# UCSD-Comp-Imaging/Nerf-Simple

Hardware: NVIDIA B200
Metric: rays/sec (64 samples/ray) render (higher is better)
Workload: dtype bf16

## Files before the change

nerf_simple_b200/csrc/mlp_chain.cuh:

```cuda
constexpr uint32_t kC_A = 0, kC_E = 2 * kABytes, kC_W = kC_E + 2 * kEBytes;
constexpr int kCStages = 4;
constexpr uint32_t kCStageBytes = 16384;
constexpr uint32_t kC_Bar = kC_W + kCStages * kCStageBytes;
constexpr uint32_t kC_Bias = kC_Bar + 256;
constexpr uint32_t kCSmemLaunch = kC_Bias + 2 * 1024;
constexpr int kCThreads = 640;
constexpr int kCProducerWarp = 16, kCMmaWarp = 17, kCStoreWarp0 = 18;
constexpr uint32_t kB_WFull = 0, kB_WPeer = 32, kB_WEmpty = 64, kB_Act = 96, kB_Acc = 112, kB_Tmem = 128, kB_Written = 136,
                   kB_StoreFree = 152;

struct TileCtx {
  int64_t tile;
  int slot;
  int half;
  int part;
  uint32_t r;
  uint32_t rowoff;
  uint32_t r7s;
  uint32_t a_img, e_img, t_lane;
  uint32_t b_img;
  const float* gf;
};
__device__ __forceinline__ uint32_t sw_off(const TileCtx& c, uint32_t kb, uint32_t j) {
  return kb * 16384u + c.rowoff + ((j << 4) ^ c.r7s);
// ... 137 lines not shown

  const int64_t PT = (p.num_tiles + 1) / 2;
  const int64_t C = num_clusters_x(), cid = cluster_id_x();
  const int64_t my_pt = (cid < PT) ? (PT - cid + C - 1) / C : 0;
  const SlabDesc* slabs = Epi::slabs();

  if (warp < 16) {
    const int slot = Epi::kSlots == 2 ? warp >> 3 : 0;
    TileCtx c;
    c.slot = slot;
    c.half = (warp >> 2) & 1;
    c.part = warp >> 2;
    c.r = (uint32_t)(warp & 3) * 32u + (uint32_t)lane;
    c.rowoff = c.r * 128u;
    c.r7s = (c.r & 7u) << 4;
    c.a_img = smem_base + kC_A + slot * kABytes;
    c.e_img = smem_base + kC_E + slot * kEBytes;
    c.t_lane = tmem_base + (((uint32_t)(warp & 3) * 32u) << 16) + (uint32_t)slot * 256u;
    c.b_img = smem_base + kC_Bias + (uint32_t)slot * 1024u;
    c.gf = reinterpret_cast<const float*>(p.packed + (Epi::kSched == kSchedFwd3 ? c_layout.f32_off3 : c_layout.f32_off));
    const uint32_t act_remote = mapa_shared(bar + kB_Act + 8 * slot, 0);
    uint32_t acc_parity = 0, free_parity = 0;
    typename Epi::State st;
    bool first_step = true;
    long long t_epi = 0, t_accw = 0, t_pro = 0, t_reclaim = 0, t_after = 0, t_stage = 0;
    auto publish = [&](bool to_mma) {
      fence_proxy_async_smem();
      tc_fence_before();
      __syncwarp();
      if (lane == 0) {
        if (Epi::kBulkStore) mbar_arrive(bar + kB_Written + 8 * slot);
        if (to_mma) mbar_arrive_cluster(act_remote);
      }
    };
    const uint32_t bias_t = threadIdx.x & 255u;
    auto fetch_bias = [&](int l) -> float { return Epi::kStageBias ? __ldg(c.gf + kF32Bias + Epi::bias_row(l) * 256 + (int)bias_t) : 0.f; };
    auto stage_bias = [&](float v) {
      if (!Epi::kStageBias) return;
      if (Epi::kSlots == 2) slot_barrier(slot); else asm volatile("bar.sync 1, 512;" ::: "memory");
      if (Epi::kSlots == 2 || threadIdx.x < 256u) asm volatile("st.shared.f32 [%0], %1;" ::"r"(c.b_img + bias_t * 4u), "f"(v) : "memory");
      if (Epi::kSlots == 2) slot_barrier(slot); else asm volatile("bar.sync 1, 512;" ::: "memory");
    };
    auto reclaim = [&]() {
      if (Epi::kBulkStore && !first_step) {
        mbar_wait(bar + kB_StoreFree + 8 * slot, free_parity, 500);
        free_parity ^= 1;
      }
      first_step = false;
    };
    Epi::init_slot(c);
    for (int64_t k = slot; k < my_pt; k += Epi::kSlots) {
      c.tile = 2 * (cid + k * C) + rank;
      if (Epi::kReverseTiles) c.tile = 2 * (PT - 1 - (cid + k * C)) + rank;
      reclaim();
      long long tq0 = 0;
      if constexpr (Epi::kHasDbg && kDevBuild) tq0 = clock64();
      const float bias0 = fetch_bias(0);
      Epi::begin_tile(p, st, c);
      publish(true);
      stage_bias(bias0);
      if constexpr (Epi::kHasDbg && kDevBuild) t_pro += clock64() - tq0;
      for (int l = 0; l < Epi::kNumLayers; ++l) {
        Epi::prefetch(p, st, c, l);
        if constexpr (Epi::kHasDbg && kDevBuild) tq0 = clock64();
        mbar_wait(bar + kB_Acc + 8 * slot, acc_parity, 100 + l);
        acc_parity ^= 1;
        tc_fence_after();
        long long tq1 = 0;
        if constexpr (Epi::kHasDbg && kDevBuild) { tq1 = clock64(); t_accw += tq1 - tq0; }
        reclaim();
        if constexpr (Epi::kHasDbg && kDevBuild) t_reclaim += clock64() - tq1;
        const float bias_next = fetch_bias(l + 1 < Epi::kNumLayers ? l + 1 : l);
        Epi::layer(p, st, c, l);
        if (Epi::kBulkStore || l + 1 < Epi::kNumLayers) publish(l + 1 < Epi::kNumLayers);
        if constexpr (Epi::kHasDbg && kDevBuild) {
          const long long tq2 = clock64();
          t_epi += tq2 - tq1;
          if ((p.dbg & 8) && threadIdx.x == 0 && rank == 0 && p.dbg_counters) {
            atomicAdd(p.dbg_counters + 16 + l, (unsigned long long)(tq2 - tq1));
            atomicAdd(p.dbg_counters + 32 + l, (unsigned long long)(tq1 - tq0));
          }
        }
        long long tq3 = 0;
        if constexpr (Epi::kHasDbg && kDevBuild) tq3 = clock64();
        if (l + 1 < Epi::kNumLayers) stage_bias(bias_next);
        long long tq4 = 0;
        if constexpr (Epi::kHasDbg && kDevBuild) { tq4 = clock64(); t_stage += tq4 - tq3; }
        Epi::after_publish(p, st, c, l);
        if constexpr (Epi::kHasDbg && kDevBuild) t_after += clock64() - tq4;
      }
    }
    if constexpr (Epi::kHasDbg && kDevBuild) {
      if ((p.dbg & 8) && threadIdx.x == 0 && rank == 0 && p.dbg_counters) {
        atomicAdd(p.dbg_counters + 4, (unsigned long long)t_epi);
        atomicAdd(p.dbg_counters + 5, (unsigned long long)t_accw);
        atomicAdd(p.dbg_counters + 6, (unsigned long long)t_pro);
        atomicAdd(p.dbg_counters + 12, (unsigned long long)t_reclaim);
        atomicAdd(p.dbg_counters + 13, (unsigned long long)t_stage);
        atomicAdd(p.dbg_counters + 14, (unsigned long long)t_after);
      }
    }
    if (Epi::kBulkStore && !first_step) mbar_wait(bar + kB_StoreFree + 8 * slot, free_parity, 501);
  } else if (warp == kCProducerWarp) {
    if (lane == 0) {
      uint32_t stage = 0, phase = 0;
      long long t_pempty = 0;
      for (int64_t pr = 0; pr * Epi::kSlots < my_pt; ++pr) {
        const int nslots = (Epi::kSlots == 2 && my_pt - 2 * pr >= 2) ? 2 : 1;
        int s0 = 0;
        for (int l = 0; l < Epi::kNumLayers; ++l) {
          int s1 = s0;
          while (!slabs[s1].last) ++s1;
          const int reps = (nslots == 2 && s1 - s0 + 1 <= kCStages) ? 1 : nslots;
          for (int rep = 0; rep < reps; ++rep) {
            for (int s = s0; s <= s1; ++s) {
              const uint32_t half = slabs[s].bytes >> 1;
              if constexpr (Epi::kHasDbg && kDevBuild) {
                const long long tp0 = clock64();
                mbar_wait(bar + kB_WEmpty + 8 * stage, phase ^ 1, 200);
                const long long tp1 = clock64();
                t_pempty += tp1 - tp0;
              } else
              mbar_wait(bar + kB_WEmpty + 8 * stage, phase ^ 1, 200);
              if (rank == 0) mbar_arrive_expect_tx(bar + kB_WFull + 8 * stage, slabs[s].bytes);
              const int32_t row0 = (int32_t)(slabs[s].off >> 7) + (int32_t)(rank * (half >> 7));
              tma_tensor2d_g2s_2cta(smem_base + kC_W + stage * kCStageBytes, half == 16384u ? &p.tmap128 : &p.tmap64, 0, row0,
// ... 83 lines not shown
  int64_t num_tiles;
  float* rgb;
  float* disp;
  float* acc;
  int64_t B;
  int sampler;
  uint64_t seed, offset;
  float tn, tf;
  const float* poses;
  int H, W;
  float f;
  int64_t ray_begin;
};
constexpr int kInCamera = 2;

__device__ __forceinline__ void load_ray_chain(const FwdEpiParams& p, int64_t ray, float (&o)[6]) {
  if (p.in_mode == kInCamera) {
    camera_ray(p.poses, p.H, p.W, p.f, p.ray_begin + ray, o);
  } else {
    const float2* q = reinterpret_cast<const float2*>(p.in0 + ray * 6);
    const float2 a = __ldg(q), b = __ldg(q + 1), c = __ldg(q + 2);
    o[0] = a.x; o[1] = a.y; o[2] = b.x; o[3] = b.y; o[4] = c.x; o[5] = c.y;
  }
}

template <bool kRender>
__device__ __forceinline__ void load_query_chain(const FwdEpiParams& p, int64_t m, float v[6], float& t) {
  if (!kRender && p.in_mode == NB200_IN_POINTS) {
    const float2* q = reinterpret_cast<const float2*>(p.in0 + m * 6);
    const float2 a = __ldg(q), b = __ldg(q + 1), c = __ldg(q + 2);
    v[0] = a.x; v[1] = a.y; v[2] = b.x; v[3] = b.y; v[4] = c.x; v[5] = c.y;
    t = 0.f;
  } else {
    const int64_t ray = p.nshift >= 0 ? (m >> p.nshift) : m / p.N;
    float o[6];
    if (kRender) {
      load_ray_chain(p, ray, o);
      t = p.sampler ? philox_sample_depth(m, (int)(m - ray * p.N), p.N, p.tn, p.tf, p.seed, p.offset) : __ldg(p.in1 + m);
    } else {
      const float2* q = reinterpret_cast<const float2*>(p.in0 + ray * 6);
      const float2 a = __ldg(q), b = __ldg(q + 1), c = __ldg(q + 2);
      o[0] = a.x; o[1] = a.y; o[2] = b.x; o[3] = b.y; o[4] = c.x; o[5] = c.y;
      t = __ldg(p.in1 + m);
    }
    const float dx = o[3], dy = o[4], dz = o[5];
    v[0] = __fadd_rn(o[0], __fmul_rn(dx, t));
    v[1] = __fadd_rn(o[1], __fmul_rn(dy, t));
    v[2] = __fadd_rn(o[2], __fmul_rn(dz, t));
    const float inv = 1.0f / sqrtf(fmaf(dz, dz, fmaf(dy, dy, dx * dx)));
    v[3] = dx * inv; v[4] = dy * inv; v[5] = dz * inv;
  }
}

template <int S>
__device__ __forceinline__ void composite_staged_ray(const FwdEpiParams& p, uint32_t stage_o, uint32_t stage_t, int ray_local,
                                                     int64_t ray, int lane) {
  constexpr int N = 32 * S;
  float4 o[S];
  float t[S];
  const uint32_t row0 = (uint32_t)(ray_local * N + lane * S);
#pragma unroll
  for (int j = 0; j < S; ++j) {
    asm volatile("ld.shared.v4.f32 {%0,%1,%2,%3}, [%4];" : "=f"(o[j].x), "=f"(o[j].y), "=f"(o[j].z), "=f"(o[j].w) : "r"(stage_o + (row0 + j) * 16u));
    asm volatile("ld.shared.f32 %0, [%1];" : "=f"(t[j]) : "r"(stage_t + (row0 + j) * 4u));
  }
  float rd[6];
  load_ray_chain(p, ray, rd);
  const float norm = unit_dir_norm(rd[3], rd[4], rd[5]);
  const float t_next_lane = __shfl_down_sync(0xffffffffu, t[0], 1);
  float a[S], pre[S];
  float run = 1.f;
#pragma unroll
  for (int j = 0; j < S; ++j) {
    const bool last = (j == S - 1 && lane == 31);
    const float tn = (j == S - 1) ? t_next_lane : t[j + 1 < S ? j + 1 : j];
    const float d = last ? 1e10f : __fsub_rn(tn, t[j]);
    const float delta = __fmul_rn(d, norm);
    const float e = transmit_factor(o[j].w, delta);
    a[j] = __fsub_rn(1.f, e);
    const float fac = __fadd_rn(__fsub_rn(1.f, a[j]), 1e-10f);
    pre[j] = run;
    run *= fac;
  }
  float pr = run;
#pragma unroll
  for (int d = 1; d < 32; d <<= 1) {
    const float v = __shfl_up_sync(0xffffffffu, pr, d);
    pr *= (lane >= d) ? v : 1.f;
  }
  float ex = __shfl_up_sync(0xffffffffu, pr, 1);
  ex = lane == 0 ? 1.f : ex;
  float sr = 0.f, sg = 0.f, sb = 0.f, sd = 0.f, sa = 0.f;
#pragma unroll
  for (int j = 0; j < S; ++j) {
    const float w = a[j] * (ex * pre[j]);
    sr = fmaf(w, o[j].x, sr); sg = fmaf(w, o[j].y, sg); sb = fmaf(w, o[j].z, sb);
    sd = fmaf(w, t[j], sd);
    sa += w;
  }
#pragma unroll
  for (int d = 16; d > 0; d >>= 1) {
    sr += __shfl_xor_sync(0xffffffffu, sr, d); sg += __shfl_xor_sync(0xffffffffu, sg, d);
    sb += __shfl_xor_sync(0xffffffffu, sb, d); sd += __shfl_xor_sync(0xffffffffu, sd, d);
    sa += __shfl_xor_sync(0xffffffffu, sa, d);
  }
  if (lane == 0) {
// ... 47 lines not shown
    if (w0 == 0x12345678u && w1 == w2 && w3 == 0x9abcdef0u) st_shared_v4(c.a_img + o, w0, w1, w2, w3);
#else
    st_shared_v4(c.a_img + o, w0, w1, w2, w3);
#endif
  }
}

#ifdef NB_PROBE_NOLDTM
#define tmem_ld16(addr, arr) do { _Pragma("unroll") for (int i_ = 0; i_ < 16; ++i_) arr[i_] = (addr) + (uint32_t)i_; } while (0)
#endif
__device__ __forceinline__ void load_bias16(const TileCtx& c, int col0, float4 (&bq)[4]) {
#pragma unroll
  for (int i = 0; i < 4; ++i)
    asm volatile("ld.shared.v4.f32 {%0,%1,%2,%3}, [%4];" : "=f"(bq[i].x), "=f"(bq[i].y), "=f"(bq[i].z), "=f"(bq[i].w) : "r"(c.b_img + (uint32_t)(col0 + 4 * i) * 4u));
}
template <bool kRelu, bool kSigma, bool kSave, int kHalf>
__device__ __forceinline__ void epi_hidden_h(const TileCtx& c, float& sigma) {
  constexpr int cbase = kHalf * 128;
  uint32_t a0[16], a1[16];
  float4 bq[4];
  tmem_ld16(c.t_lane + cbase, a0);
#pragma unroll
  for (int q = 0; q < 8; q += 2) {
    load_bias16(c, cbase + q * 16, bq);
    tmem_ld_wait();
    tmem_ld16(c.t_lane + cbase + (q + 1) * 16, a1);
    epi_cols16<kRelu, kSigma, kSave>(c, a0, cbase + q * 16, bq, sigma);
    load_bias16(c, cbase + (q + 1) * 16, bq);
    tmem_ld_wait();
    if (q + 2 < 8) tmem_ld16(c.t_lane + cbase + (q + 2) * 16, a0);
    epi_cols16<kRelu, kSigma, kSave>(c, a1, cbase + (q + 1) * 16, bq, sigma);
  }
}
template <bool kRelu, bool kSigma, bool kSave>
__device__ __forceinline__ void epi_hidden(const TileCtx& c, float& sigma) {
  if (c.half == 0) epi_hidden_h<kRelu, kSigma, kSave, 0>(c, sigma);
  else epi_hidden_h<kRelu, kSigma, kSave, 1>(c, sigma);
}
#ifdef NB_PROBE_NOLDTM
#undef tmem_ld16
#endif

template <bool kSave, bool kRender = false, bool kFold = false>
struct FwdEpi {
  static_assert(!(kSave && kRender), "the fused render kernel is inference only");
  using Params = FwdEpiParams;
  static constexpr bool kHasDbg = true;
  static constexpr bool kBulkStore = kSave;
  static constexpr int kSched = kFold ? kSchedFwdFold : kSchedFwd;
  static constexpr bool kStageBias = true;
  static constexpr int kSlots = 2;
  static constexpr int kNumLayers = kFold ? kNumFoldLayers : kNumMmaLayers;
  static constexpr bool kReverseTiles = false;
  __device__ static constexpr int ml_of(int l) { return (kFold && l == 8) ? 9 : l; }
  __device__ static constexpr int bias_row(int l) { return (kFold && l == 8) ? kFoldBiasRow : l; }
  struct State {
    float v[6];
    float sigma;
    float t;
    int64_t m_raw;
    bool row_valid;
  };
  __device__ static const SlabDesc* slabs() { return kFold ? c_layout.fwdf : c_layout.fwd; }
  __device__ static void init_slot(const TileCtx&) {}

  __device__ static void prefetch(const Params&, State&, const TileCtx&, int) {}

  __device__ static void after_publish(const Params& p, State& st, const TileCtx& c, int l) {
    const int ml = ml_of(l);
    if (ml == 5) {
      if (c.half == 0) encode_row<kLd, 0, 2>(st.v + 3, c.e_img, c.r, nullptr);
      else encode_row<kLd, 2, 4>(st.v + 3, c.e_img, c.r, nullptr);
#pragma unroll
      for (uint32_t i = threadIdx.x & 255u; i < kTabFloats; i += 256u) {
        const float v = __ldg(c.gf + (i < kTabWC1 ? kF32WSig + (int)i
                                                  : (i < kTabBC1 ? kF32WC1 + (int)(i - kTabWC1) : (i < kTabBSig ? kF32BC1 + (int)(i - kTabBC1) : kF32BSig))));
        asm volatile("st.shared.f32 [%0], %1;" ::"r"(c.e_img + tab_off(i)), "f"(v) : "memory");
      }
    }
    if (!kSave || ml < 0 || ml == 8) return;
    const int64_t T = p.num_tiles;
    if (ml < 8) {
      uint8_t* row = p.saved + mask_tensor_off(ml, T) + (size_t)c.tile * 4096 + ((size_t)(c.half * 128) + c.r) * 16;
      uint32_t m[4];
#pragma unroll
      for (int q = 0; q < 4; ++q) {
        const uint32_t kb = (uint32_t)(c.half * 2 + (q >> 1)), j0 = (uint32_t)(q & 1) * 4u;
        uint32_t f[2] = {0u, 0u};
#pragma unroll
        for (int j = 0; j < 4; ++j) {
          uint32_t w0, w1, w2, w3;
          asm volatile("ld.shared.v4.b32 {%0,%1,%2,%3}, [%4];" : "=r"(w0), "=r"(w1), "=r"(w2), "=r"(w3) : "r"(c.a_img + sw_off(c, kb, j0 + j)));
          add_pair_flags(f[j >> 1], w0, 4 * (j & 1)); add_pair_flags(f[j >> 1], w1, 4 * (j & 1) + 1);
          add_pair_flags(f[j >> 1], w2, 4 * (j & 1) + 2); add_pair_flags(f[j >> 1], w3, 4 * (j & 1) + 3);
        }
        m[q] = fold_mask16(f[0]) | (fold_mask16(f[1]) << 16);
      }
      *reinterpret_cast<uint4*>(row) = make_uint4(m[0], m[1], m[2], m[3]);
    } else {
      uint8_t* row = p.saved + mask_tensor_off(8, T) + (size_t)c.tile * 2048 + ((size_t)(c.half * 128) + c.r) * 8;
      uint32_t m[2];
#pragma unroll
      for (int q = 0; q < 2; ++q) {
        uint32_t f[2] = {0u, 0u};
#pragma unroll
        for (int j = 0; j < 4; ++j) {
          uint32_t w0, w1, w2, w3;
          asm volatile("ld.shared.v4.b32 {%0,%1,%2,%3}, [%4];" : "=r"(w0), "=r"(w1), "=r"(w2), "=r"(w3)
                       : "r"(c.a_img + sw_off(c, (uint32_t)c.half, (uint32_t)(q * 4 + j))));
          add_pair_flags(f[j >> 1], w0, 4 * (j & 1)); add_pair_flags(f[j >> 1], w1, 4 * (j & 1) + 1);
          add_pair_flags(f[j >> 1], w2, 4 * (j & 1) + 2); add_pair_flags(f[j >> 1], w3, 4 * (j & 1) + 3);
        }
        m[q] = fold_mask16(f[0]) | (fold_mask16(f[1]) << 16);
      }
      *reinterpret_cast<uint2*>(row) = make_uint2(m[0], m[1]);
    }
  }

  __device__ static void begin_tile(const Params& p, State& st, const TileCtx& c) {
    st.m_raw = c.tile * kTileM + c.r;
    st.row_valid = st.m_raw < p.M;
    load_query_chain<kRender>(p, st.row_valid ? st.m_raw : p.M - 1, st.v, st.t);
    st.sigma = 0.f;
    if (c.half == 0) encode_row<kLp, 0, 4>(st.v, c.e_img, c.r, nullptr);
    else encode_row<kLp, 4, 8>(st.v, c.e_img, c.r, nullptr);
  }

  __device__ static void store_tile(const Params& p, const TileCtx& c, int l) {
    const int64_t T = p.num_tiles;
    const int ml = ml_of(l);
    if (ml == -1) tma_bulk_s2g(p.saved + saved_tensor_off(10, T) + (size_t)c.tile * 16384, c.e_img, 16384);
    else if (ml < 9) tma_bulk_s2g(p.saved + saved_tensor_off(ml, T) + (size_t)c.tile * 65536, c.a_img, 65536);
    else tma_bulk_s2g(p.saved + saved_tensor_off(9, T) + (size_t)c.tile * 32768, c.a_img, 32768);
    if (ml == 6) tma_bulk_s2g(p.saved + saved_tensor_off(11, T) + (size_t)c.tile * 16384, c.e_img, 16384);
  }

  __device__ static void layer(const Params& p, State& st, const TileCtx& c, int l) {
    const int ml = ml_of(l);
    if (ml < 9) {
      if (ml == 7) epi_hidden<true, true, kSave>(c, st.sigma);
      else if (ml == 8) epi_hidden<false, false, kSave>(c, st.sigma);
      else epi_hidden<true, false, kSave>(c, st.sigma);
    } else {
      float rgb[3] = {0.f, 0.f, 0.f};
#pragma unroll 1
      for (int q = 0; q < 2; ++q) {
        const int col0 = c.half * 64 + q * 32;
        uint32_t a[32];
        tmem_ld32(c.t_lane + col0, a);
        tmem_ld_wait();
#pragma unroll
        for (int j = 0; j < 4; ++j) {
          float x[8], b[8];
          asm volatile("ld.shared.v4.f32 {%0,%1,%2,%3}, [%4];" : "=f"(b[0]), "=f"(b[1]), "=f"(b[2]), "=f"(b[3]) : "r"(c.b_img + (uint32_t)(col0 + 8 * j) * 4u));
          asm volatile("ld.shared.v4.f32 {%0,%1,%2,%3}, [%4];" : "=f"(b[4]), "=f"(b[5]), "=f"(b[6]), "=f"(b[7]) : "r"(c.b_img + (uint32_t)(col0 + 8 * j + 4) * 4u));
#pragma unroll
          for (int e = 0; e < 8; ++e) x[e] = fmaxf(__uint_as_float(a[8 * j + e]) + b[e], 0.f);
#pragma unroll
          for (int k = 0; k < 3; ++k) {
            const float4 w0 = tab_ld4(c.e_img, kTabWC1 + (uint32_t)(k * 128 + col0 + 8 * j)), w1 = tab_ld4(c.e_img, kTabWC1 + (uint32_t)(k * 128 + col0 + 8 * j + 4));
            rgb[k] = fmaf(x[0], w0.x, rgb[k]); rgb[k] = fmaf(x[1], w0.y, rgb[k]); rgb[k] = fmaf(x[2], w0.z, rgb[k]); rgb[k] = fmaf(x[3], w0.w, rgb[k]);
            rgb[k] = fmaf(x[4], w1.x, rgb[k]); rgb[k] = fmaf(x[5], w1.y, rgb[k]); rgb[k] = fmaf(x[6], w1.z, rgb[k]); rgb[k] = fmaf(x[7], w1.w, rgb[k]);
          }
          if (kSave) {
            const uint32_t w0 = pack_bf16x2(x[0], x[1]), w1 = pack_bf16x2(x[2], x[3]), w2 = pack_bf16x2(x[4], x[5]),
                           w3 = pack_bf16x2(x[6], x[7]);
            st_shared_v4(c.a_img + sw_off(c, (uint32_t)c.half, (uint32_t)(q * 4 + j)), w0, w1, w2, w3);
          }
        }
      }
      const uint32_t xaddr = c.e_img + c.r * 16u;
      if (c.half == 1) st_shared_v4(xaddr, __float_as_uint(rgb[0]), __float_as_uint(rgb[1]), __float_as_uint(rgb[2]), __float_as_uint(st.sigma));
      slot_barrier(c.slot);
      if (c.half == 0) {
        float4 o;
        asm volatile("ld.shared.v4.f32 {%0,%1,%2,%3}, [%4];" : "=f"(o.x), "=f"(o.y), "=f"(o.z), "=f"(o.w) : "r"(xaddr));
        const float4 hb = tab_ld4(c.e_img, kTabBC1);
        const float4 res = make_float4(rgb[0] + o.x + hb.x, rgb[1] + o.y + hb.y, rgb[2] + o.z + hb.z, st.sigma + o.w + hb.w);
        if (kRender) {
          st_shared_v4(c.a_img + c.r * 16u, __float_as_uint(res.x), __float_as_uint(res.y), __float_as_uint(res.z), __float_as_uint(res.w));
          asm volatile("st.shared.f32 [%0], %1;" ::"r"(c.a_img + 2048u + c.r * 4u), "f"(st.t) : "memory");
        } else if (st.row_valid) {
          reinterpret_cast<float4*>(p.out)[st.m_raw] = res;
        }
      }
      slot_barrier(c.slot);
      if (kRender) {
        const int wq = (int)(threadIdx.x >> 5) & 7, nr = kTileM / p.N;
        const int64_t ray = c.tile * nr + wq;
        if (wq < nr && ray < p.B) {
          const int lane = (int)threadIdx.x & 31;
          if (p.N == 64) composite_staged_ray<2>(p, c.a_img, c.a_img + 2048u, wq, ray, lane);
          else if (p.N == 128) composite_staged_ray<4>(p, c.a_img, c.a_img + 2048u, wq, ray, lane);
          else composite_staged_ray<1>(p, c.a_img, c.a_img + 2048u, wq, ray, lane);
        }
      }
    }
  }
};

__device__ __forceinline__ void split_hi_lo(float x0, float x1, uint32_t& hi, uint32_t& lo) {
  hi = pack_bf16x2(x0, x1);
  lo = pack_bf16x2(x0 - __uint_as_float(hi << 16), x1 - __uint_as_float(hi & 0xFFFF0000u));
}
template <int L, int J0, int J1>
__device__ __forceinline__ void encode_row3(const float* x, uint32_t img_hi, uint32_t img_lo, uint32_t r) {
  float f[64];
#pragma unroll
  for (int i = 0; i < 64; ++i) f[i] = 0.f;
#pragma unroll
  for (int c = 0; c < 3; ++c) {
    f[c] = x[c];
#pragma unroll
    for (int i = 0; i < L; ++i) {
      float sv, cv;
      sincosf(ldexpf(x[c], i), &sv, &cv);
      f[3 + c * 2 * L + 2 * i] = sv;
      f[3 + c * 2 * L + 2 * i + 1] = cv;
    }
  }
#pragma unroll
  for (int j = J0; j < J1; ++j) {
    uint32_t h[4], l[4];
#pragma unroll
    for (int e = 0; e < 4; ++e) split_hi_lo(f[8 * j + 2 * e], f[8 * j + 2 * e + 1], h[e], l[e]);
    st_shared_v4(img_hi + sw128_off(r, j), h[0], h[1], h[2], h[3]);
    st_shared_v4(img_lo + sw128_off(r, j), l[0], l[1], l[2], l[3]);
  }
}

struct FwdEpi3 {
  using Params = FwdEpiParams;
  static constexpr bool kHasDbg = false;
  static constexpr bool kBulkStore = false;
  static constexpr int kSched = kSchedFwd3;
  static constexpr bool kStageBias = true;
  static constexpr int kSlots = 1;
  static constexpr int kNumLayers = kNumMmaLayers;
  static constexpr bool kReverseTiles = false;
  struct State {
    float v[6];
    float sigma;
    int64_t m_raw;
    bool row_valid;
  };
  __device__ static const SlabDesc* slabs() { return c_layout.fwd3; }
  __device__ static constexpr int bias_row(int l) { return l; }
  __device__ static void init_slot(const TileCtx&) {}
  __device__ static void prefetch(const Params&, State&, const TileCtx&, int) {}
  __device__ static void after_publish(const Params&, State&, const TileCtx&, int) {}
  __device__ static void store_tile(const Params&, const TileCtx&, int) {}

  __device__ static void encode(const float* x, const TileCtx& c, bool dirs) {
    const uint32_t hi = c.e_img, lo = c.e_img + kEBytes;
    if (!dirs) {
      if (c.part == 0) encode_row3<kLp, 0, 2>(x, hi, lo, c.r);
      else if (c.part == 1) encode_row3<kLp, 2, 4>(x, hi, lo, c.r);
      else if (c.part == 2) encode_row3<kLp, 4, 6>(x, hi, lo, c.r);
      else encode_row3<kLp, 6, 8>(x, hi, lo, c.r);
    } else {
      if (c.part == 0) encode_row3<kLd, 0, 2>(x, hi, lo, c.r);
      else if (c.part == 1) encode_row3<kLd, 2, 4>(x, hi, lo, c.r);
      else if (c.part == 2) encode_row3<kLd, 4, 6>(x, hi, lo, c.r);
      else encode_row3<kLd, 6, 8>(x, hi, lo, c.r);
    }
  }

  __device__ static void begin_tile(const Params& p, State& st, const TileCtx& c) {
    st.m_raw = c.tile * kTileM + c.r;
    st.row_valid = st.m_raw < p.M;
    float t;
    load_query_chain<false>(p, st.row_valid ? st.m_raw : p.M - 1, st.v, t);
    st.sigma = 0.f;
    encode(st.v, c, false);
  }

  __device__ static void layer(const Params& p, State& st, const TileCtx& c, int ml) {
    if (ml == 5) encode(st.v + 3, c, true);
    const uint32_t a_hi = c.a_img, a_lo = c.a_img + kABytes;
    if (ml < 9) {
      const int cbase = c.part * 64;
      const float* ws = c.gf + kF32WSig;
#pragma unroll 1
      for (int q = 0; q < 4; ++q) {
        const int col0 = cbase + q * 16;
        uint32_t a[16];
        float4 bq[4];
        tmem_ld16(c.t_lane + col0, a);
        load_bias16(c, col0, bq);
        tmem_ld_wait();
        const uint32_t kb = (uint32_t)col0 >> 6, j0 = ((uint32_t)col0 >> 3) & 7u;
#pragma unroll
// ... 28 lines not shown
      float rgb[3] = {0.f, 0.f, 0.f};
#pragma unroll
      for (int q = 0; q < 2; ++q) {
        float4 bq[4];
        load_bias16(c, col0 + 16 * q, bq);
#pragma unroll
        for (int g = 0; g < 4; ++g) {
          const float b[4] = {bq[g].x, bq[g].y, bq[g].z, bq[g].w};
          float x[4];
#pragma unroll
          for (int e = 0; e < 4; ++e) x[e] = fmaxf(__uint_as_float(a[16 * q + 4 * g + e]) + b[e], 0.f);
#pragma unroll
          for (int k = 0; k < 3; ++k) {
            const float4 wv = __ldg(w4 + k * 32 + 4 * q + g);
            rgb[k] = fmaf(x[0], wv.x, rgb[k]); rgb[k] = fmaf(x[1], wv.y, rgb[k]);
            rgb[k] = fmaf(x[2], wv.z, rgb[k]); rgb[k] = fmaf(x[3], wv.w, rgb[k]);
          }
        }
      }
      const uint32_t xaddr = c.e_img + ((uint32_t)c.part * 128u + c.r) * 16u;
      if (c.part != 0) st_shared_v4(xaddr, __float_as_uint(rgb[0]), __float_as_uint(rgb[1]), __float_as_uint(rgb[2]), __float_as_uint(st.sigma));
      asm volatile("bar.sync 1, 512;" ::: "memory");
      if (c.part == 0) {
        float4 acc = make_float4(rgb[0], rgb[1], rgb[2], st.sigma);
#pragma unroll
        for (int q = 1; q < 4; ++q) {
          float4 o;
          asm volatile("ld.shared.v4.f32 {%0,%1,%2,%3}, [%4];" : "=f"(o.x), "=f"(o.y), "=f"(o.z), "=f"(o.w) : "r"(c.e_img + ((uint32_t)q * 128u + c.r) * 16u));
          acc.x += o.x; acc.y += o.y; acc.z += o.z; acc.w += o.w;
        }
        if (st.row_valid)
          reinterpret_cast<float4*>(p.out)[st.m_raw] = make_float4(acc.x + __ldg(c.gf + kF32BC1), acc.y + __ldg(c.gf + kF32BC1 + 1), acc.z + __ldg(c.gf + kF32BC1 + 2),
                                                                   acc.w + __ldg(c.gf + kF32BSig));
      }
      asm volatile("bar.sync 1, 512;" ::: "memory");
    }
  }
};

#ifndef NB_DG_L2HINT
#define NB_DG_L2HINT 2
#endif
template <bool kFold>
struct DgradEpi {
  using Params = BwdParams;
  static constexpr bool kHasDbg = false;
  static constexpr bool kBulkStore = true;
  static constexpr int kSched = kSchedBwd;
  static constexpr bool kStageBias = false;
  static constexpr int kSlots = 2;
  static constexpr int kNumLayers = kFold ? 8 : 9;
  static constexpr int kBl0 = kFold ? 2 : 1;
  static constexpr bool kReverseTiles = true;
  struct State { float4 g; uint4 mask; };
  __device__ static const SlabDesc* slabs() { return kFold ? c_layout.bwdf : c_layout.bwd; }
  __device__ static constexpr int bias_row(int l) { return l; }
  __device__ static void after_publish(const Params&, State&, const TileCtx&, int) {}
  __device__ static void init_slot(const TileCtx& c) {
    for (uint32_t i = threadIdx.x & 255u; i < 640u; i += 256u)
      asm volatile("st.shared.f32 [%0], %1;" ::"r"(c.e_img + i * 4u), "f"(__ldg(c.gf + (i < 256u ? kF32WSig + (int)i : kF32WC1 + (int)(i - 256u)))) : "memory");
    slot_barrier(c.slot);
  }
  __device__ static __forceinline__ float4 head_ld4(const TileCtx& c, uint32_t i) {
    float4 v;
    asm volatile("ld.shared.v4.f32 {%0,%1,%2,%3}, [%4];" : "=f"(v.x), "=f"(v.y), "=f"(v.z), "=f"(v.w) : "r"(c.e_img + i * 4u));
    return v;
  }

  __device__ static void prefetch(const Params& p, State& st, const TileCtx& c, int l) {
    const int bl = l + kBl0;
    if (bl >= 2)
      st.mask = __ldg(reinterpret_cast<const uint4*>(p.saved + mask_tensor_off(9 - bl, p.num_tiles) + (size_t)c.tile * 4096 +
                                                     ((size_t)(c.half * 128) + c.r) * 16));
  }

  __device__ static void begin_tile(const Params& p, State& st, const TileCtx& c) {
    const int64_t T = p.num_tiles;
    const int64_t m_raw = c.tile * kTileM + c.r;
    st.g = make_float4(0.f, 0.f, 0.f, 0.f);
    if (m_raw < p.M) st.g = __ldg(reinterpret_cast<const float4*>(p.d_out) + m_raw);
    const uint2 cbits = __ldg(reinterpret_cast<const uint2*>(p.saved + mask_tensor_off(8, T) + (size_t)c.tile * 2048 +
                                                             ((size_t)(c.half * 128) + c.r) * 8));
    const uint32_t kb = (uint32_t)c.half;
#pragma unroll
    for (int j = 0; j < 8; ++j) {
      const uint32_t o = sw_off(c, kb, j);
      const uint32_t field = ((j < 4 ? cbits.x : cbits.y) >> (16 * ((j >> 1) & 1))) & 0xFFFFu;
      const int k0 = 4 * (j & 1);
      const uint32_t col = (uint32_t)(c.half * 64 + j * 8);
      float x[8];
      {
        const float4 a0 = head_ld4(c, 256u + col), a1 = head_ld4(c, 256u + col + 4u);
        x[0] = st.g.x * a0.x; x[1] = st.g.x * a0.y; x[2] = st.g.x * a0.z; x[3] = st.g.x * a0.w;
        x[4] = st.g.x * a1.x; x[5] = st.g.x * a1.y; x[6] = st.g.x * a1.z; x[7] = st.g.x * a1.w;
        const float4 b0 = head_ld4(c, 384u + col), b1 = head_ld4(c, 384u + col + 4u);
        x[0] = fmaf(st.g.y, b0.x, x[0]); x[1] = fmaf(st.g.y, b0.y, x[1]); x[2] = fmaf(st.g.y, b0.z, x[2]); x[3] = fmaf(st.g.y, b0.w, x[3]);
        x[4] = fmaf(st.g.y, b1.x, x[4]); x[5] = fmaf(st.g.y, b1.y, x[5]); x[6] = fmaf(st.g.y, b1.z, x[6]); x[7] = fmaf(st.g.y, b1.w, x[7]);
        const float4 c0 = head_ld4(c, 512u + col), c1 = head_ld4(c, 512u + col + 4u);
        x[0] = fmaf(st.g.z, c0.x, x[0]); x[1] = fmaf(st.g.z, c0.y, x[1]); x[2] = fmaf(st.g.z, c0.z, x[2]); x[3] = fmaf(st.g.z, c0.w, x[3]);
        x[4] = fmaf(st.g.z, c1.x, x[4]); x[5] = fmaf(st.g.z, c1.y, x[5]); x[6] = fmaf(st.g.z, c1.z, x[6]); x[7] = fmaf(st.g.z, c1.w, x[7]);
      }
      const uint32_t w0 = pack_bf16x2(x[0], x[1]) & pair_mask_word(field, k0), w1 = pack_bf16x2(x[2], x[3]) & pair_mask_word(field, k0 + 1),
                     w2 = pack_bf16x2(x[4], x[5]) & pair_mask_word(field, k0 + 2), w3 = pack_bf16x2(x[6], x[7]) & pair_mask_word(field, k0 + 3);
      st_shared_v4(c.a_img + o, w0, w1, w2, w3);
    }
  }
// ... 60 lines not shown
```

nerf_simple_b200/csrc/mlp_tc.cu:

```cuda
#include <cuda.h>
#include <stdlib.h>
#include <string.h>

#include <mutex>
#include <utility>

#include "common.cuh"
#include "stream_common.cuh"
#include "tc_common.cuh"

namespace nb200 {
using namespace tc;

constexpr int kNumMmaLayers = 10;
constexpr int kMaxSlabs = 48;
constexpr int kNumFoldLayers = kNumMmaLayers - 1;
constexpr int kLayerFold = 100;
constexpr int kFoldBiasRow = 10;

struct SlabDesc {
  uint32_t off;
  uint32_t bytes;
  uint16_t n;
  uint16_t wcol0;
// ... 511 lines not shown
      snprintf(g_last_cuda_error, sizeof(g_last_cuda_error), "cuTensorMapEncodeTiled failed (%d)", (int)r);
      return NB200_ERR_CUDA;
    }
  }
  t.packed = packed;
  t.dev = dev;
  t.rows = rows;
  *out = t;
  return NB200_OK;
}

static int chain_grid(int64_t T) {
  const int64_t PT = (T + 1) / 2;
  const int64_t want = (PT + 1) / 2;
  const int64_t maxc = sm_count() / 2;
  const int64_t clusters = want < maxc ? (want > 0 ? want : 1) : maxc;
  return (int)(2 * clusters);
}

int tc_forward(int in_mode, const float* in0, const float* in1, int64_t M, int N, const void* packed,
               float* out, void* saved, void*, size_t, int fold, cudaStream_t s) {
  NB_TRY_RC(check_arch());
  NB_TRY_RC(ensure_layout());
  NB_TRY_RC(ensure_attr(&DeviceState::attr_fwd, []() -> int {
    NB_CUDA_CHECK(cudaFuncSetAttribute(chain_kernel<FwdEpi<false>>, cudaFuncAttributeMaxDynamicSharedMemorySize,
                                       (int)kCSmemLaunch));
    NB_CUDA_CHECK(cudaFuncSetAttribute(chain_kernel<FwdEpi<true>>, cudaFuncAttributeMaxDynamicSharedMemorySize,
                                       (int)kCSmemLaunch));
    NB_CUDA_CHECK(cudaFuncSetAttribute(chain_kernel<FwdEpi<false, false, true>>, cudaFuncAttributeMaxDynamicSharedMemorySize,
                                       (int)kCSmemLaunch));
    NB_CUDA_CHECK(cudaFuncSetAttribute(chain_kernel<FwdEpi<true, false, true>>, cudaFuncAttributeMaxDynamicSharedMemorySize,
                                       (int)kCSmemLaunch));
    return NB200_OK;
  }));
  const int64_t T = saved ? train_tiles(M) : ceil_div64(M, kTileM);
  FwdEpiParams p;
  TmapPair tm;
  NB_TRY_RC(get_tmaps(packed, &tm));
  p.tmap128 = tm.m128; p.tmap64 = tm.m64;
  p.dbg = 0;
  p.dbg_counters = nullptr;
#ifdef NB200_DEV
  { const char* e = getenv("NB200_DBG"); p.dbg = e ? atoi(e) : 0; }
  if (p.dbg & 8) {
    static unsigned long long* ctr = nullptr;
    if (!ctr) { cudaMalloc(&ctr, 512); cudaMemset(ctr, 0, 512); }
    unsigned long long h[64];
    cudaMemcpy(h, ctr, 512, cudaMemcpyDeviceToHost);
    printf("nb200 dbg: mma-warp cycles wait_act=%llu total=%llu | epilogue warp 0: layers=%llu wait_acc=%llu prologue=%llu | producer wait_empty=%llu | epilogue warp 0: reclaim (inside layers)=%llu stage_bias=%llu after_publish=%llu\n",
           h[0], h[3], h[4], h[5], h[6], h[7], h[12], h[13], h[14]);
    printf("nb200 dbg: epilogue warp 0 per layer, busy | wait_acc (share of total):");
    for (int l = 0; l < 10; ++l) printf(" L%d %.1f|%.1f", l, 100.0 * (double)h[16 + l] / (double)(h[3] ? h[3] : 1), 100.0 * (double)h[32 + l] / (double)(h[3] ? h[3] : 1));
    printf("\n");
    cudaMemset(ctr, 0, 512);
    p.dbg_counters = ctr;
  }
#endif
  p.in_mode = in_mode; p.in0 = in0; p.in1 = in1; p.M = M; p.N = N;
  p.nshift = (N > 0 && (N & (N - 1)) == 0) ? __builtin_ctz((unsigned)N) : -1;
  p.packed = reinterpret_cast<const uint8_t*>(packed);
  p.out = out; p.saved = reinterpret_cast<uint8_t*>(saved);
  p.num_tiles = T;
  const int grid = chain_grid(T);
  if (saved && fold)
    chain_kernel<FwdEpi<true, false, true>><<<grid, kCThreads, kCSmemLaunch, s>>>(p);
  else if (saved)
    chain_kernel<FwdEpi<true>><<<grid, kCThreads, kCSmemLaunch, s>>>(p);
  else if (fold)
    chain_kernel<FwdEpi<false, false, true>><<<grid, kCThreads, kCSmemLaunch, s>>>(p);
  else
    chain_kernel<FwdEpi<false>><<<grid, kCThreads, kCSmemLaunch, s>>>(p);
  NB_LAUNCH_CHECK("chain_kernel<FwdEpi>");
  return NB200_OK;
}

int tc_forward_x3(int in_mode, const float* in0, const float* in1, int64_t M, int N, const void* packed, float* out,
                  cudaStream_t s) {
  NB_TRY_RC(check_arch());
  NB_TRY_RC(ensure_layout());
  NB_TRY_RC(ensure_attr(&DeviceState::attr_x3, []() -> int {
    NB_CUDA_CHECK(cudaFuncSetAttribute(chain_kernel<FwdEpi3>, cudaFuncAttributeMaxDynamicSharedMemorySize, (int)kCSmemLaunch));
    return NB200_OK;
  }));
  const int64_t T = ceil_div64(M, kTileM);
  FwdEpiParams p;
  memset(&p, 0, sizeof(p));
  TmapPair tm;
  NB_TRY_RC(get_tmaps(packed, &tm, 1));
  p.tmap128 = tm.m128; p.tmap64 = tm.m64;
  p.in_mode = in_mode; p.in0 = in0; p.in1 = in1; p.M = M; p.N = N;
  p.nshift = (N > 0 && (N & (N - 1)) == 0) ? __builtin_ctz((unsigned)N) : -1;
  p.packed = reinterpret_cast<const uint8_t*>(packed);
  p.out = out;
  p.num_tiles = T;
  const int64_t PT = (T + 1) / 2, maxc = sm_count() / 2;
  const int grid = (int)(2 * (PT < maxc ? PT : maxc));
  chain_kernel<FwdEpi3><<<grid, kCThreads, kCSmemLaunch, s>>>(p);
  NB_LAUNCH_CHECK("chain_kernel<FwdEpi3>");
  return NB200_OK;
}

int tc_render(const float* rays, const float* poses, int H, int W, float f, int64_t ray_begin, const float* ts, uint64_t seed,
              uint64_t offset, int64_t B, int N, float tn, float tf, const void* packed, float* rgb, float* disp, float* acc,
              int fold, cudaStream_t s) {
  NB_TRY_RC(check_arch());
  NB_TRY_RC(ensure_layout());
// ... 137 lines not shown
```

nerf_simple_b200/csrc/tc_common.cuh:

```cuda
#pragma once
#include <cuda_bf16.h>
#include <stdint.h>

namespace nb200 {
namespace tc {

__device__ __forceinline__ uint32_t smem_u32(const void* p) {
  return static_cast<uint32_t>(__cvta_generic_to_shared(p));
}

__device__ __forceinline__ void mbar_init(uint32_t bar, uint32_t count) {
  asm volatile("mbarrier.init.shared::cta.b64 [%0], %1;" ::"r"(bar), "r"(count) : "memory");
}
__device__ __forceinline__ void fence_mbar_init() {
  asm volatile("fence.mbarrier_init.release.cluster;" ::: "memory");
}
__device__ __forceinline__ void mbar_arrive(uint32_t bar) {
  asm volatile("mbarrier.arrive.shared::cta.b64 _, [%0];" ::"r"(bar) : "memory");
}
__device__ __forceinline__ void mbar_arrive_expect_tx(uint32_t bar, uint32_t bytes) {
  asm volatile("mbarrier.arrive.expect_tx.shared::cta.b64 _, [%0], %1;" ::"r"(bar), "r"(bytes) : "memory");
}
__device__ __forceinline__ bool mbar_try_wait(uint32_t bar, uint32_t parity) {
  uint32_t ok;
// ... 3 lines not shown
      "selp.u32 %0, 1, 0, p;\n\t}"
      : "=r"(ok)
      : "r"(bar), "r"(parity)
      : "memory");
  return ok != 0;
}
__device__ __forceinline__ uint64_t global_timer_ns() {
  uint64_t t;
  asm volatile("mov.u64 %0, %%globaltimer;" : "=l"(t));
  return t;
}
__device__ __forceinline__ void mbar_wait(uint32_t bar, uint32_t parity, int tag) {
  if (mbar_try_wait(bar, parity)) return;
  const uint64_t t0 = global_timer_ns();
  uint32_t it = 0;
  while (!mbar_try_wait(bar, parity)) {
    if ((++it & 0xFFFu) == 0u && global_timer_ns() - t0 > 4000000000ull) {
      printf("nb200: mbarrier wait timed out (block %d thread %d tag %d parity %u)\n", blockIdx.x,
             threadIdx.x, tag, parity);
      __trap();
    }
  }
}

__device__ __forceinline__ void tma_bulk_g2s(uint32_t dst_smem, const void* src_gmem, uint32_t bytes,
                                             uint32_t bar) {
  asm volatile(
      "cp.async.bulk.shared::cluster.global.mbarrier::complete_tx::bytes [%0], [%1], %2, [%3];" ::"r"(dst_smem),
      "l"(src_gmem), "r"(bytes), "r"(bar)
      : "memory");
}

__device__ __forceinline__ void tma_tensor2d_g2s_2cta(uint32_t dst_smem, const void* tmap, int32_t c0, int32_t c1,
                                                      uint32_t bar_cluster) {
  asm volatile(
      "cp.async.bulk.tensor.2d.cta_group::2.shared::cluster.global.mbarrier::complete_tx::bytes [%0], [%1, {%2, %3}], [%4];" ::"r"(dst_smem),
      "l"(tmap), "r"(c0), "r"(c1), "r"(bar_cluster)
      : "memory");
}

__device__ __forceinline__ void tma_bulk_s2g(void* dst_gmem, uint32_t src_smem, uint32_t bytes) {
  asm volatile("cp.async.bulk.global.shared::cta.bulk_group [%0], [%1], %2;" ::"l"(dst_gmem), "r"(src_smem), "r"(bytes)
               : "memory");
  asm volatile("cp.async.bulk.commit_group;" ::: "memory");
}
__device__ __forceinline__ void tma_bulk_store_wait_read() {
  asm volatile("cp.async.bulk.wait_group.read 0;" ::: "memory");
}

__device__ __forceinline__ void tma_prefetch_l2(const void* gmem, uint32_t bytes) {
  asm volatile("cp.async.bulk.prefetch.L2.global [%0], %1;" ::"l"(gmem), "r"(bytes) : "memory");
}

__device__ __forceinline__ uint64_t l2_policy_evict_last() {
  uint64_t p;
  asm volatile("createpolicy.fractional.L2::evict_last.b64 %0, 1.0;" : "=l"(p));
  return p;
}
__device__ __forceinline__ uint64_t l2_policy_evict_first() {
  uint64_t p;
  asm volatile("createpolicy.fractional.L2::evict_first.b64 %0, 1.0;" : "=l"(p));
  return p;
}
__device__ __forceinline__ void tma_prefetch_l2_hint(const void* gmem, uint32_t bytes, uint64_t policy) {
  asm volatile("cp.async.bulk.prefetch.L2.global.L2::cache_hint [%0], %1, %2;" ::"l"(gmem), "r"(bytes), "l"(policy) : "memory");
}
__device__ __forceinline__ void tma_bulk_s2g_hint(void* dst_gmem, uint32_t src_smem, uint32_t bytes, uint64_t policy) {
  asm volatile("cp.async.bulk.global.shared::cta.bulk_group.L2::cache_hint [%0], [%1], %2, %3;" ::"l"(dst_gmem), "r"(src_smem),
               "r"(bytes), "l"(policy)
               : "memory");
  asm volatile("cp.async.bulk.commit_group;" ::: "memory");
}

__device__ __forceinline__ void fence_proxy_async_smem() {
  asm volatile("fence.proxy.async.shared::cta;" ::: "memory");
}
__device__ __forceinline__ void tc_fence_before() {
  asm volatile("tcgen05.fence::before_thread_sync;" ::: "memory");
}
__device__ __forceinline__ void tc_fence_after() {
  asm volatile("tcgen05.fence::after_thread_sync;" ::: "memory");
}

__device__ __forceinline__ void tmem_alloc(uint32_t dst_smem, uint32_t ncols) {
  asm volatile("tcgen05.alloc.cta_group::1.sync.aligned.shared::cta.b32 [%0], %1;" ::"r"(dst_smem), "r"(ncols)
               : "memory");
  asm volatile("tcgen05.relinquish_alloc_permit.cta_group::1.sync.aligned;" ::: "memory");
}
__device__ __forceinline__ void tmem_dealloc(uint32_t taddr, uint32_t ncols) {
  asm volatile("tcgen05.dealloc.cta_group::1.sync.aligned.b32 %0, %1;" ::"r"(taddr), "r"(ncols) : "memory");
}
__device__ __forceinline__ void tmem_ld32(uint32_t taddr, uint32_t (&r)[32]) {
  asm volatile(
      "tcgen05.ld.sync.aligned.32x32b.x32.b32 "
      "{%0,%1,%2,%3,%4,%5,%6,%7,%8,%9,%10,%11,%12,%13,%14,%15,"
      "%16,%17,%18,%19,%20,%21,%22,%23,%24,%25,%26,%27,%28,%29,%30,%31}, [%32];"
      : "=r"(r[0]), "=r"(r[1]), "=r"(r[2]), "=r"(r[3]), "=r"(r[4]), "=r"(r[5]), "=r"(r[6]), "=r"(r[7]),
        "=r"(r[8]), "=r"(r[9]), "=r"(r[10]), "=r"(r[11]), "=r"(r[12]), "=r"(r[13]), "=r"(r[14]), "=r"(r[15]),
        "=r"(r[16]), "=r"(r[17]), "=r"(r[18]), "=r"(r[19]), "=r"(r[20]), "=r"(r[21]), "=r"(r[22]), "=r"(r[23]),
        "=r"(r[24]), "=r"(r[25]), "=r"(r[26]), "=r"(r[27]), "=r"(r[28]), "=r"(r[29]), "=r"(r[30]), "=r"(r[31])
      : "r"(taddr)
      : "memory");
}
__device__ __forceinline__ void tmem_ld16(uint32_t taddr, uint32_t (&r)[16]) {
  asm volatile(
      "tcgen05.ld.sync.aligned.32x32b.x16.b32 "
// ... 144 lines not shown
```

Baseline: 20.17 million.

## Overlap next tile's query load and encode with current tile's final epilogue

Restructures the forward epilogue loop so that after the last layer's MMA epilogue, the next tile's inputs are loaded, encoded and published to the MMA warp before the previous tile's output combine, compositing and mask save run. The final-layer half exchange moves to dedicated shared-memory scratch so the encode buffers can be reused early, and the next-next tile's inputs are prefetched into L2. The aim is to hide the tile-boundary prologue latency, where the tensor cores would otherwise sit idle. It adds complexity around shared-memory reuse and ordering, and extra scratch traffic.

```diff
diff --git a/nerf_simple_b200/csrc/mlp_chain.cuh b/nerf_simple_b200/csrc/mlp_chain.cuh
--- a/nerf_simple_b200/csrc/mlp_chain.cuh
+++ b/nerf_simple_b200/csrc/mlp_chain.cuh
@@ -213,14 +213,19 @@
     for (int64_t k = slot; k < my_pt; k += Epi::kSlots) {
       c.tile = 2 * (cid + k * C) + rank;
       if (Epi::kReverseTiles) c.tile = 2 * (PT - 1 - (cid + k * C)) + rank;
-      reclaim();
       long long tq0 = 0;
-      if constexpr (Epi::kHasDbg && kDevBuild) tq0 = clock64();
-      const float bias0 = fetch_bias(0);
-      Epi::begin_tile(p, st, c);
-      publish(true);
-      stage_bias(bias0);
-      if constexpr (Epi::kHasDbg && kDevBuild) t_pro += clock64() - tq0;
+      if (!Epi::kOverlapBoundary || k == slot) {
+        reclaim();
+        if constexpr (Epi::kHasDbg && kDevBuild) tq0 = clock64();
+        const float bias0 = fetch_bias(0);
+        Epi::begin_tile(p, st, c);
+        publish(true);
+        if constexpr (Epi::kOverlapBoundary) {
+          if (k + Epi::kSlots < my_pt) Epi::prefetch_tile(p, c, c.tile + 2 * Epi::kSlots * C);
+        }
+        stage_bias(bias0);
+        if constexpr (Epi::kHasDbg && kDevBuild) t_pro += clock64() - tq0;
+      }
       for (int l = 0; l < Epi::kNumLayers; ++l) {
         Epi::prefetch(p, st, c, l);
         if constexpr (Epi::kHasDbg && kDevBuild) tq0 = clock64();
@@ -233,6 +238,39 @@
         if constexpr (Epi::kHasDbg && kDevBuild) t_reclaim += clock64() - tq1;
         const float bias_next = fetch_bias(l + 1 < Epi::kNumLayers ? l + 1 : l);
         Epi::layer(p, st, c, l);
+        if constexpr (Epi::kOverlapBoundary) {
+          if (l + 1 == Epi::kNumLayers) {
+            if (Epi::kBulkStore) publish(false);
+            slot_barrier(slot);
+            const long long tq2 = kDevBuild ? clock64() : 0;
+            if constexpr (kDevBuild) {
+              t_epi += tq2 - tq1;
+              if ((p.dbg & 8) && threadIdx.x == 0 && rank == 0 && p.dbg_counters) {
+                atomicAdd(p.dbg_counters + 16 + l, (unsigned long long)(tq2 - tq1));
+                atomicAdd(p.dbg_counters + 32 + l, (unsigned long long)(tq1 - tq0));
+              }
+            }
+            if (k + Epi::kSlots < my_pt) {
+              c.tile += 2 * Epi::kSlots * C;
+              Epi::begin_tile(p, st, c);
+              reclaim();
+              publish(true);
+              const long long tq3 = kDevBuild ? clock64() : 0;
+              if constexpr (kDevBuild) t_pro += tq3 - tq2;
+              if (k + 2 * Epi::kSlots < my_pt) Epi::prefetch_tile(p, c, c.tile + 2 * Epi::kSlots * C);
+              const float bias0 = fetch_bias(0);
+              Epi::end_tile(p, c, c.tile - 2 * Epi::kSlots * C);
+              stage_bias(bias0);
+              if constexpr (kDevBuild) {
+                if ((p.dbg & 8) && threadIdx.x == 0 && rank == 0 && p.dbg_counters)
+                  atomicAdd(p.dbg_counters + 10, (unsigned long long)(clock64() - tq3));
+              }
+            } else {
+              Epi::end_tile(p, c, c.tile);
+            }
+            continue;
+          }
+        }
         if (Epi::kBulkStore || l + 1 < Epi::kNumLayers) publish(l + 1 < Epi::kNumLayers);
         if constexpr (Epi::kHasDbg && kDevBuild) {
           const long long tq2 = clock64();
@@ -422,6 +460,11 @@
   }
 }
 
+__device__ __forceinline__ void prefetch_l2_floats(const float* base, int64_t first, int64_t last, int lane) {
+  const int64_t i = first + 32 * (int64_t)lane;
+  if (i <= last + 31) prefetch_l2_line(base + (i < last ? i : last));
+}
+
 template <int S>
 __device__ __forceinline__ void composite_staged_ray(const FwdEpiParams& p, uint32_t stage_o, uint32_t stage_t, int ray_local,
                                                      int64_t ray, int lane) {
@@ -575,6 +618,7 @@
   static constexpr int kSlots = 2;
   static constexpr int kNumLayers = kFold ? kNumFoldLayers : kNumMmaLayers;
   static constexpr bool kReverseTiles = false;
+  static constexpr bool kOverlapBoundary = true;
   __device__ static constexpr int ml_of(int l) { return (kFold && l == 8) ? 9 : l; }
   __device__ static constexpr int bias_row(int l) { return (kFold && l == 8) ? kFoldBiasRow : l; }
   struct State {
@@ -601,7 +645,7 @@
         asm volatile("st.shared.f32 [%0], %1;" ::"r"(c.e_img + tab_off(i)), "f"(v) : "memory");
       }
     }
-    if (!kSave || ml < 0 || ml == 8) return;
+    if (!kSave || ml < 0 || ml >= 8) return;
     const int64_t T = p.num_tiles;
     if (ml < 8) {
       uint8_t* row = p.saved + mask_tensor_off(ml, T) + (size_t)c.tile * 4096 + ((size_t)(c.half * 128) + c.r) * 16;
@@ -620,8 +664,35 @@
         m[q] = fold_mask16(f[0]) | (fold_mask16(f[1]) << 16);
       }
       *reinterpret_cast<uint4*>(row) = make_uint4(m[0], m[1], m[2], m[3]);
-    } else {
-      uint8_t* row = p.saved + mask_tensor_off(8, T) + (size_t)c.tile * 2048 + ((size_t)(c.half * 128) + c.r) * 8;
+    }
+  }
+
+  static constexpr uint32_t kXchg = 3u * 16384u, kXchgHalf0 = kXchg + 2048u, kXchgBias = kXchg + 4096u;
+
+  __device__ static void end_tile(const Params& p, const TileCtx& c, int64_t tile) {
+    const int64_t m_raw = tile * kTileM + c.r;
+    if (c.half == 0) {
+      float4 s, o, hb;
+      asm volatile("ld.shared.v4.f32 {%0,%1,%2,%3}, [%4];" : "=f"(s.x), "=f"(s.y), "=f"(s.z), "=f"(s.w) : "r"(c.a_img + kXchgHalf0 + c.r * 16u));
+      asm volatile("ld.shared.v4.f32 {%0,%1,%2,%3}, [%4];" : "=f"(o.x), "=f"(o.y), "=f"(o.z), "=f"(o.w) : "r"(c.a_img + kXchg + c.r * 16u));
+      asm volatile("ld.shared.v4.f32 {%0,%1,%2,%3}, [%4];" : "=f"(hb.x), "=f"(hb.y), "=f"(hb.z), "=f"(hb.w) : "r"(c.a_img + kXchgBias));
+      const float4 res = make_float4(s.x + o.x + hb.x, s.y + o.y + hb.y, s.z + o.z + hb.z, s.w + o.w + hb.w);
+      if (kRender) st_shared_v4(c.a_img + c.r * 16u, __float_as_uint(res.x), __float_as_uint(res.y), __float_as_uint(res.z), __float_as_uint(res.w));
+      else if (m_raw < p.M) reinterpret_cast<float4*>(p.out)[m_raw] = res;
+    }
+    if (kRender) {
+      slot_barrier(c.slot);
+      const int wq = (int)(threadIdx.x >> 5) & 7, nr = kTileM / p.N;
+      const int64_t ray = tile * nr + wq;
+      if (wq < nr && ray < p.B) {
+        const int lane = (int)threadIdx.x & 31;
+        if (p.N == 64) composite_staged_ray<2>(p, c.a_img, c.a_img + 2048u, wq, ray, lane);
+        else if (p.N == 128) composite_staged_ray<4>(p, c.a_img, c.a_img + 2048u, wq, ray, lane);
+        else composite_staged_ray<1>(p, c.a_img, c.a_img + 2048u, wq, ray, lane);
+      }
+    }
+    if (kSave) {
+      uint8_t* row = p.saved + mask_tensor_off(8, p.num_tiles) + (size_t)tile * 2048 + ((size_t)(c.half * 128) + c.r) * 8;
       uint32_t m[2];
 #pragma unroll
       for (int q = 0; q < 2; ++q) {
@@ -640,13 +711,43 @@
     }
   }
 
+  __device__ static void prefetch_tile(const Params& p, const TileCtx& c, int64_t tile) {
+    const int64_t m0 = tile * kTileM;
+    if (c.half != 0 || c.r >= 32u || m0 >= p.M) return;
+    const int64_t m1 = (m0 + kTileM < p.M ? m0 + kTileM : p.M) - 1;
+    if (!kRender && p.in_mode == NB200_IN_POINTS) {
+      prefetch_l2_floats(p.in0, 6 * m0, 6 * m1 + 5, (int)c.r);
+      return;
+    }
+    if (!(kRender && p.sampler)) prefetch_l2_floats(p.in1, m0, m1, (int)c.r);
+    if (!(kRender && p.in_mode == kInCamera)) {
+      const int64_t r0 = p.nshift >= 0 ? (m0 >> p.nshift) : m0 / p.N, r1 = p.nshift >= 0 ? (m1 >> p.nshift) : m1 / p.N;
+      prefetch_l2_floats(p.in0, 6 * r0, 6 * r1 + 5, (int)c.r);
+    }
+  }
+
   __device__ static void begin_tile(const Params& p, State& st, const TileCtx& c) {
+#ifdef NB200_DEV
+    const long long tb0 = clock64();
+#endif
     st.m_raw = c.tile * kTileM + c.r;
     st.row_valid = st.m_raw < p.M;
     load_query_chain<kRender>(p, st.row_valid ? st.m_raw : p.M - 1, st.v, st.t);
     st.sigma = 0.f;
+#ifdef NB200_DEV
+    long long tb1;
+    asm volatile("{\n\t.reg .pred q;\n\tsetp.eq.f32 q, %1, %1;\n\t@q mov.u64 %0, %%clock64;\n\t@!q mov.u64 %0, %%clock64;\n\t}"
+                 : "=l"(tb1) : "f"(st.v[0] + st.v[5]));
+#endif
     if (c.half == 0) encode_row<kLp, 0, 4>(st.v, c.e_img, c.r, nullptr);
     else encode_row<kLp, 4, 8>(st.v, c.e_img, c.r, nullptr);
+#ifdef NB200_DEV
+    if ((p.dbg & 8) && threadIdx.x == 0 && (c.tile & 1) == 0 && p.dbg_counters) {
+      atomicAdd(p.dbg_counters + 8, (unsigned long long)(tb1 - tb0));
+      atomicAdd(p.dbg_counters + 9, (unsigned long long)(clock64() - tb1));
+      atomicAdd(p.dbg_counters + 11, 1ull);
+    }
+#endif
   }
 
   __device__ static void store_tile(const Params& p, const TileCtx& c, int l) {
@@ -692,32 +793,13 @@
           }
         }
       }
-      const uint32_t xaddr = c.e_img + c.r * 16u;
-      if (c.half == 1) st_shared_v4(xaddr, __float_as_uint(rgb[0]), __float_as_uint(rgb[1]), __float_as_uint(rgb[2]), __float_as_uint(st.sigma));
-      slot_barrier(c.slot);
-      if (c.half == 0) {
-        float4 o;
-        asm volatile("ld.shared.v4.f32 {%0,%1,%2,%3}, [%4];" : "=f"(o.x), "=f"(o.y), "=f"(o.z), "=f"(o.w) : "r"(xaddr));
+      st_shared_v4(c.a_img + (c.half == 0 ? kXchgHalf0 : kXchg) + c.r * 16u, __float_as_uint(rgb[0]), __float_as_uint(rgb[1]),
+                   __float_as_uint(rgb[2]), __float_as_uint(st.sigma));
+      if (c.half == 1 && c.r == 0) {
         const float4 hb = tab_ld4(c.e_img, kTabBC1);
-        const float4 res = make_float4(rgb[0] + o.x + hb.x, rgb[1] + o.y + hb.y, rgb[2] + o.z + hb.z, st.sigma + o.w + hb.w);
-        if (kRender) {
-          st_shared_v4(c.a_img + c.r * 16u, __float_as_uint(res.x), __float_as_uint(res.y), __float_as_uint(res.z), __float_as_uint(res.w));
-          asm volatile("st.shared.f32 [%0], %1;" ::"r"(c.a_img + 2048u + c.r * 4u), "f"(st.t) : "memory");
-        } else if (st.row_valid) {
-          reinterpret_cast<float4*>(p.out)[st.m_raw] = res;
-        }
-      }
-      slot_barrier(c.slot);
-      if (kRender) {
-        const int wq = (int)(threadIdx.x >> 5) & 7, nr = kTileM / p.N;
-        const int64_t ray = c.tile * nr + wq;
-        if (wq < nr && ray < p.B) {
-          const int lane = (int)threadIdx.x & 31;
-          if (p.N == 64) composite_staged_ray<2>(p, c.a_img, c.a_img + 2048u, wq, ray, lane);
-          else if (p.N == 128) composite_staged_ray<4>(p, c.a_img, c.a_img + 2048u, wq, ray, lane);
-          else composite_staged_ray<1>(p, c.a_img, c.a_img + 2048u, wq, ray, lane);
-        }
-      }
+        st_shared_v4(c.a_img + kXchgBias, __float_as_uint(hb.x), __float_as_uint(hb.y), __float_as_uint(hb.z), __float_as_uint(hb.w));
+      }
+      if (kRender && c.half == 0) asm volatile("st.shared.f32 [%0], %1;" ::"r"(c.a_img + 2048u + c.r * 4u), "f"(st.t) : "memory");
     }
   }
 };
@@ -761,6 +843,7 @@
   static constexpr int kSlots = 1;
   static constexpr int kNumLayers = kNumMmaLayers;
   static constexpr bool kReverseTiles = false;
+  static constexpr bool kOverlapBoundary = false;
   struct State {
     float v[6];
     float sigma;
@@ -895,6 +978,7 @@
   static constexpr int kNumLayers = kFold ? 8 : 9;
   static constexpr int kBl0 = kFold ? 2 : 1;
   static constexpr bool kReverseTiles = true;
+  static constexpr bool kOverlapBoundary = false;
   struct State { float4 g; uint4 mask; };
   __device__ static const SlabDesc* slabs() { return kFold ? c_layout.bwdf : c_layout.bwd; }
   __device__ static constexpr int bias_row(int l) { return l; }
diff --git a/nerf_simple_b200/csrc/mlp_tc.cu b/nerf_simple_b200/csrc/mlp_tc.cu
--- a/nerf_simple_b200/csrc/mlp_tc.cu
+++ b/nerf_simple_b200/csrc/mlp_tc.cu
@@ -587,6 +587,10 @@
     printf("nb200 dbg: epilogue warp 0 per layer, busy | wait_acc (share of total):");
     for (int l = 0; l < 10; ++l) printf(" L%d %.1f|%.1f", l, 100.0 * (double)h[16 + l] / (double)(h[3] ? h[3] : 1), 100.0 * (double)h[32 + l] / (double)(h[3] ? h[3] : 1));
     printf("\n");
+    const double nt = (double)(h[11] ? h[11] : 1);
+    printf("nb200 dbg: per tile, epilogue thread 0: tiles=%llu query_load=%.0f encode=%.0f prologue=%.0f boundary_tail=%.0f | "
+           "L0 wait_acc=%.0f busy=%.0f | L8 wait_acc=%.0f busy=%.0f | mma-warp total=%.0f\n",
+           h[11], h[8] / nt, h[9] / nt, h[6] / nt, h[10] / nt, h[32] / nt, h[16] / nt, h[40] / nt, h[24] / nt, h[3] / nt);
     cudaMemset(ctr, 0, 512);
     p.dbg_counters = ctr;
   }
diff --git a/nerf_simple_b200/csrc/tc_common.cuh b/nerf_simple_b200/csrc/tc_common.cuh
--- a/nerf_simple_b200/csrc/tc_common.cuh
+++ b/nerf_simple_b200/csrc/tc_common.cuh
@@ -79,6 +79,10 @@
   asm volatile("cp.async.bulk.prefetch.L2.global [%0], %1;" ::"l"(gmem), "r"(bytes) : "memory");
 }
 
+__device__ __forceinline__ void prefetch_l2_line(const void* gmem) {
+  asm volatile("prefetch.global.L2 [%0];" ::"l"(gmem));
+}
+
 __device__ __forceinline__ uint64_t l2_policy_evict_last() {
   uint64_t p;
   asm volatile("createpolicy.fractional.L2::evict_last.b64 %0, 1.0;" : "=l"(p));
```

Result: no change. 20.21 million, median of 6 (+0.2%).
